# heathsc/bs_call

Measured on AMD Instinct MI355X. Metric: genome positions called/sec, higher is better.
Workload: dtype f64

## Files before the change

### bs_call_amd/csrc/prepdev.hip

```cpp
#include <hip/hip_runtime.h>
#include <stdint.h>

#include "../../include/bscall_amd.h"

#define FLT_QUAL 63u

struct bsc_prep_plan {
  uint64_t src;
  uint64_t ms;
  uint32_t rl0;
  uint32_t w0, wl;
  uint32_t nm;
  uint32_t mark_l, mark_r;
  uint32_t out_len;
  uint32_t present;
  uint32_t trim_l, trim_r;
};

struct bsc_prep_desc {
  uint64_t srcw;
  uint32_t pk;
  int32_t pc;
};
#define PD_PRESENT 1u
// ... 45 lines not shown
  {                                                                                                                                    \
    const uint32_t q = ((w_) >> 2) & 0x3f3f3f3fu;                                                                                      \
    const uint32_t nz = ((q ^ 0x3f3f3f3fu) + 0x7f7f7f7fu) & 0x80808080u;  \
    n += (uint32_t)__popc(nz);                                                                                                         \
    tot = __builtin_amdgcn_sad_u8(q & ((nz >> 7) * 0xffu), 0u, tot);                                       \
  }
  for (; i + 16u <= hi; i += 16u) {
    uint4 v;
    __builtin_memcpy(&v, sp + i, 16);
    MQ_DWORD(v.x) MQ_DWORD(v.y) MQ_DWORD(v.z) MQ_DWORD(v.w)
  }
  for (; i + 4u <= hi; i += 4u) MQ_DWORD(d_ld32(sp + i))
#undef MQ_DWORD
  for (; i < hi; i++) {
    const uint32_t q = (uint32_t)sp[i] >> 2;
    if (q != FLT_QUAL) {
      tot += q;
      n++;
    }
  }
  return n > 0 ? tot / n : 0;
}

__global__ __launch_bounds__(256) void bsc_prep_plan_kernel(const bsc_raw_template *__restrict__ raw, uint32_t nr, const uint8_t *__restrict__ seq,
                                                            uint64_t seq_bytes, const bsc_misms *__restrict__ misms_in, uint64_t n_misms_in,
                                                            bsc_prep_params par, bsc_misms *__restrict__ ms_work,
                                                            bsc_prep_plan *__restrict__ plan, bsc_prep_desc *__restrict__ desc,
                                                            unsigned long long *__restrict__ out_len,
                                                            bsc_template *__restrict__ tpl_out, unsigned long long *__restrict__ cnt,
                                                            uint32_t *__restrict__ max_pos1) {
  const uint32_t ti = blockIdx.x * 256u + threadIdx.x;
  unsigned long long n_clip = 0, n_overlap = 0;
  uint32_t err = 0;
  if (ti < nr) {
    const bsc_raw_template t = raw[ti];
    bsc_prep_plan P[2];
    prep_rd rd[2];
    uint32_t nm[2];
    bsc_misms *ms[2];
    bool edited[2] = {false, false};
    uint32_t pos[2] = {t.pos[0], t.pos[1]};
    if (t.orientation > 1) err = PE_ORI;
#pragma unroll
    for (int k = 0; k < 2 && !err; k++) {
      if (t.len[k] && (t.off[k] > seq_bytes || t.len[k] > seq_bytes - t.off[k])) err = PE_READ + (uint32_t)k;
      else if (t.n_misms[k] && (t.misms_off[k] > n_misms_in || t.n_misms[k] > n_misms_in - t.misms_off[k])) err = PE_LIST + (uint32_t)k;
    }
    if (!err) {
      const int msk = t.orientation == 0 ? 0 : 1;
#pragma unroll
      for (int k = 0; k < 2; k++) {
        const int side = k ^ msk;
        const uint32_t rl = t.len[k];
        const int32_t lt = side ? par.left_trim[1] : par.left_trim[0], rt = side ? par.right_trim[1] : par.right_trim[0];
        P[k].src = t.off[k];
        P[k].ms = t.misms_off[k];
        P[k].rl0 = rl;
        P[k].mark_l = lt > 0 ? ((uint32_t)lt < rl ? (uint32_t)lt : rl) : 0u;
        P[k].mark_r = rt > 0 ? ((uint32_t)rt < rl ? (uint32_t)rt : rl) : 0u;
        P[k].present = rl != 0;
        P[k].trim_l = P[k].trim_r = 0;
        rd[k].w0 = 0;
        rd[k].wl = rl;
        nm[k] = t.n_misms[k];
        ms[k] = ms_work + t.misms_off[k];
        for (uint32_t z = 0; z < nm[k]; z++) ms[k][z] = misms_in[t.misms_off[k] + z];
// ... 174 lines not shown
          }
          m->position = ix1;
        }
        P[k].w0 = rd[k].w0;
        P[k].wl = rl;
        P[k].nm = nm[k];
        P[k].out_len = rl + adj;
      }
    }
    if (err) {
#pragma unroll
      for (int k = 0; k < 2; k++) {
        P[k].src = P[k].ms = 0;
        P[k].rl0 = P[k].w0 = P[k].wl = P[k].nm = P[k].mark_l = P[k].mark_r = P[k].out_len = P[k].present = P[k].trim_l = P[k].trim_r = 0;
      }
      atomicMin(&cnt[0], ((unsigned long long)ti << 8) | err);
      n_clip = n_overlap = 0;
    }
#pragma unroll
    for (int k = 0; k < 2; k++) {
      bsc_prep_desc d;
      const uint32_t ol = P[k].out_len;
      d.srcw = P[k].src + P[k].w0;
      const uint32_t ml = P[k].mark_l > P[k].w0 ? (P[k].mark_l - P[k].w0 < ol ? P[k].mark_l - P[k].w0 : ol) : 0u;
      const uint32_t keep = P[k].rl0 - P[k].mark_r;
      const uint32_t hr = keep > P[k].w0 ? (keep - P[k].w0 < ol ? keep - P[k].w0 : ol) : 0u;
      const bool ed = edited[k] && !err;
      const bool slow = ol != 0 && (ed || hr < ol || ol < 4u || ol >= 0xfffffu || ml >= 256u);
      d.pk = (ol < 0xfffffu ? ol : 0xfffffu) | ((ml & 0xffu) << 20) |
             (((P[k].present ? PD_PRESENT : 0u) | (ed ? PD_EDITED : 0u) | (slow ? PD_SLOW : 0u)) << 28);
      d.pc = k ? (int32_t)(P[k].wl + P[k].trim_r) - 1 : (int32_t)P[k].trim_l;
      desc[2u * ti + (uint32_t)k] = d;
      if (slow) plan[2u * ti + (uint32_t)k] = P[k];
    }
    if (max_pos1) {
      int32_t max_pos = 0;
#pragma unroll
      for (int k = 0; k < 2; k++)
        if (P[k].present) {
          const int32_t mpos = k ? (int32_t)(P[k].wl + P[k].trim_r) - 1 : (int32_t)(P[k].trim_l + P[k].wl);
          if (mpos > max_pos) max_pos = mpos;
        }
      max_pos1[ti] = err ? 0u : (uint32_t)max_pos + 1u;
    }
    out_len[2u * ti] = P[0].out_len;
    out_len[2u * ti + 1u] = P[1].out_len;
    bsc_template o;
    o.pos[0] = pos[0];
    o.pos[1] = pos[1];
    o.len[0] = P[0].out_len;
    o.len[1] = P[1].out_len;
    o.off[0] = o.off[1] = 0;
    o.mapq[0] = t.mapq[0];
    o.mapq[1] = t.mapq[1];
    o.orientation = t.orientation;
    o.bs_strand = t.bs_strand;
    o.flags = 0;
    tpl_out[ti] = o;
  }
  for (int o = 32; o > 0; o >>= 1) {
    n_clip += __shfl_xor(n_clip, o);
    n_overlap += __shfl_xor(n_overlap, o);
  }
  if ((threadIdx.x & 63u) == 0) {
    unsigned long long *slot = cnt + PREP_CNT_WORDS + (blockIdx.x & (PREP_CNT_SLOTS - 1u)) * 8u;
    if (n_clip) atomicAdd(&slot[0], n_clip);
    if (n_overlap) atomicAdd(&slot[1], n_overlap);
  }
}

__device__ static __forceinline__ uint32_t d_marked(const uint8_t *sp, uint32_t i, uint32_t rl0, uint32_t mark_l, uint32_t mark_r) {
  const bool in_r = i >= rl0 - mark_r;
  const uint32_t b = sp[(in_r && 2u * i > rl0 - 1u) ? rl0 - 1u - i : i];
  return (i < mark_l || in_r) ? (b & 3u) | (FLT_QUAL << 2) : (uint32_t)sp[i];
}

struct bsc_prep_prof {
  const uint8_t *ref;
  uint32_t x, n_ref, cap, used0;
  const uint32_t *used_scan;
  unsigned long long *table;
};
__device__ static const uint8_t PROF_REF[64] = {
    0, 0, 0, 0, 0, 0, 0, 0, 0, 0, 0, 8, 0, 0, 0, 0, 0, 4, 4, 0, 4, 0, 0, 0, 0, 0, 0, 8, 0, 0, 0, 0,
    0, 0, 0, 8, 0, 0, 0, 0, 0, 0, 0, 0, 0, 0, 0, 0, 0, 0, 0, 0, 0, 0, 0, 0, 0, 0, 0, 0, 0, 0, 0, 0};
__device__ static __forceinline__ uint32_t d_profile_base(uint32_t bs_strand, uint32_t c) {
  const uint32_t q = c >> 2;
  if (q < 20u  || q >= FLT_QUAL || bs_strand > 2u) return 0u;
  return ((bs_strand == 0 ? 0x7A6Bu : (bs_strand == 1 ? 0x5A4Bu : 0x7869u)) >> (4u * (c & 3u))) & 15u;
}

#define PREP_WAVES 4
#define PREP_BATCH 4u
#define PROF_LDS 512u

__device__ static __forceinline__ void d_prof_base(const bsc_prep_prof &F, uint32_t *s_prof, uint32_t strand, uint32_t used_t, int64_t v,
                                                   int32_t orig, uint32_t byte) {
  const uint32_t xx = d_profile_base(strand, byte);
  if (xx && v + 1 < (int64_t)F.n_ref) {
    const uint32_t ra = v >= 1 ? F.ref[v - 1] : 0u, rb = v >= 0 ? F.ref[v] : 0u, rc = F.ref[v + 1];
    const uint32_t m_before = PROF_REF[((ra << 3) | rb) & 63u], m_after = PROF_REF[((rb << 3) | rc) & 63u];
    if ((((xx & m_after) | ((xx & m_before) >> 1)) >> 2) & 1u) {
      const uint32_t ix = (uint32_t)(orig + 1);
      if (ix < used_t && ix < F.cap) {
        if (ix < PROF_LDS) atomicAdd(&s_prof[(xx & 3u) * PROF_LDS + ix], 1u);
        else atomicAdd(&F.table[(uint64_t)ix * 4u + (xx & 3u)], 1ull);
      }
    }
  }
}

__device__ static __forceinline__ uint32_t d_bcast(uint32_t v, uint32_t l) { return (uint32_t)__builtin_amdgcn_readlane((int)v, (int)l); }
__device__ static __forceinline__ unsigned long long d_bcast64(unsigned long long v, uint32_t l) {
  return (unsigned long long)d_bcast((uint32_t)v, l) | ((unsigned long long)d_bcast((uint32_t)(v >> 32), l) << 32);
}
__device__ static __forceinline__ uint32_t d_ld32(const uint8_t *p) {
  uint32_t v;
  __builtin_memcpy(&v, p, 4);
  return v;
}
__device__ static __forceinline__ void d_st32(uint8_t *p, uint32_t v) { __builtin_memcpy(p, &v, 4); }

struct prep_slow_ret {
  uint32_t c63, cge;
  uint32_t walked;
};

__device__ static __forceinline__ uint32_t prep_slow_src(const bsc_prep_plan &P, const bsc_misms *__restrict__ ms, bool edited, uint32_t j, bool &pad) {
  uint32_t s = j;
  pad = false;
  if (edited) {
    for (uint32_t z = P.nm; z-- > 0;) {
      const bsc_misms m = ms[z];
      if (m.type == BSC_MISMS_INS) {
        if (s >= m.position) {
          if (s - m.position < m.size) {
            pad = true;
            break;
          }
          s -= m.size;
        }
      } else if (m.type == BSC_MISMS_DEL) {
        if (s >= m.position) s += m.size;
      }
    }
  }
  return s;
}

__device__ __noinline__ static prep_slow_ret prep_slow_read(const bsc_prep_plan *__restrict__ plan_r, uint32_t flags, uint8_t *__restrict__ dp,
                                                            const uint8_t *__restrict__ seq, const bsc_misms *__restrict__ ms_work, uint32_t mq) {
  const unsigned lane = threadIdx.x & 63u;
  prep_slow_ret r = {0u, 0u, 0u};
  const bsc_prep_plan P = *plan_r;
  const uint8_t *const sp = seq + P.src;
  const bool edited = (flags & PD_EDITED) != 0;
  if (edited) {
    for (uint32_t s0 = 0; s0 < P.wl; s0 += 64u) {
      const uint32_t s = s0 + lane;
      if (s < P.wl) {
        const uint32_t q = d_marked(sp, P.w0 + s, P.rl0, P.mark_l, P.mark_r) >> 2;
        r.c63 += q == FLT_QUAL;
        r.cge += q >= mq;
      }
    }
  }
  const bsc_misms *const ms = ms_work + P.ms;
  bool walked = false;
  for (uint32_t j0 = 0; j0 < P.out_len; j0 += 64u) {
    const uint32_t j = j0 + lane;
    if (j < P.out_len) {
      bool pad;
      const uint32_t s = prep_slow_src(P, ms, edited, j, pad);
      const uint32_t byte = pad ? 0u : d_marked(sp, P.w0 + s, P.rl0, P.mark_l, P.mark_r);
      const uint32_t q = byte >> 2;
      if (!edited) {
        r.c63 += q == FLT_QUAL;
        r.cge += q >= mq;
      }
      walked |= q != 0 && q != FLT_QUAL;
      dp[j] = (uint8_t)byte;
    }
  }
  r.walked = __any(walked) ? 1u : 0u;
  return r;
}

__global__ __launch_bounds__(64 * PREP_WAVES) void bsc_prep_copy_kernel(const bsc_prep_plan *__restrict__ plan,
                                                                        const bsc_prep_desc *__restrict__ desc, uint32_t nr,
                                                                        const uint8_t *__restrict__ seq, const bsc_misms *__restrict__ ms_work,
                                                                        const unsigned long long *__restrict__ out_off, int32_t min_qual,
                                                                        bsc_template *__restrict__ tpl_out, uint8_t *__restrict__ seq_out,
                                                                        uint64_t seq_out_cap, unsigned long long *__restrict__ cnt) {
  const unsigned lane = threadIdx.x & 63u, lane4 = lane * 4u;
  const uint32_t wave = (uint32_t)__builtin_amdgcn_readfirstlane((int)(blockIdx.x * PREP_WAVES + (threadIdx.x >> 6)));
  const uint32_t n_waves = gridDim.x * PREP_WAVES;
  const uint32_t mq = min_qual < 0 ? 0u : (min_qual > 64 ? 64u : (uint32_t)min_qual), mq4 = mq * 0x01010101u;
  unsigned long long l_total = 0, l_bases = 0;
  uint32_t c63 = 0, cge = 0, l_reads = 0;
  const uint32_t n_reads2 = 2u * nr, n_groups = (n_reads2 + 63u) / 64u;
  for (uint32_t g = wave; g < n_groups; g += n_waves) {
    const uint32_t g0 = g * 64u, n = n_reads2 - g0 < 64u ? n_reads2 - g0 : 64u;
    const uint32_t ri = g0 + (lane < n ? lane : 0u), my_ti = ri >> 1, my_k = ri & 1u;
    bsc_prep_desc L = desc[ri];
    const unsigned long long l_off = out_off[ri];
    if (lane >= n) L.pk = 0;
    if (lane < n) {
      const uint32_t fl = L.pk >> 28;
      uint32_t ol = L.pk & 0xfffffu, wl = ol;
      if (fl & PD_SLOW) {
        ol = plan[ri].out_len;
        wl = plan[ri].wl;
      }
      tpl_out[my_ti].off[my_k] = l_off;
      if (l_off > seq_out_cap || seq_out_cap - l_off < ol) {
        atomicMin(&cnt[0], ((unsigned long long)my_ti << 8) | PE_CAP);
        L.pk &= 0xf0000000u;
      }
      l_total += (fl & PD_EDITED) ? wl : ol;
      if (fl & PD_PRESENT) {
        l_reads++;
        l_bases += wl;
      }
    }
    enum : uint32_t { KIND_LEAN = 1u, KIND_FAST = 2u, KIND_SLOW = 3u };
    const uint32_t my_len = L.pk & 0xfffffu, my_ml = (L.pk >> 20) & 0xffu;
    const uint32_t my_kind = my_len == 0 ? 0u : ((L.pk >> 28) & PD_SLOW ? KIND_SLOW : ((my_len <= 256u && my_ml == 0) ? KIND_LEAN : KIND_FAST));
    const uint32_t l_ctl = (L.pk & 0x0fffffffu) | (my_kind << 28) | (((L.pk >> 28) & PD_EDITED) ? 1u << 30 : 0u);
    const bool my_fetch = my_kind == KIND_LEAN || my_kind == KIND_FAST;
    const unsigned long long l_src = my_fetch ? (unsigned long long)(seq + L.srcw) - (unsigned long long)desc : 0ull;
    unsigned long long walked_mask = 0;
    const unsigned long long obase = d_bcast64(l_off, 0);
    const unsigned long long m_w0 = __ballot(my_kind == KIND_LEAN && my_len >= 16u && my_len <= 128u);
    const unsigned long long sbase = m_w0 ? d_bcast64(L.srcw, (uint32_t)__builtin_ctzll(m_w0)) : 0ull;
// ... 59 lines not shown
        if (ml + 3u > base) {
          const uint32_t nmk = act && ml > o ? (ml - o < 4u ? ml - o : 4u) : 0u;
          const uint32_t mm = nmk >= 4u ? 0xffffffffu : (1u << (8u * nmk)) - 1u;
          w = (w & ~mm) | (((w & 0x03030303u) | 0xfcfcfcfcu) & mm);
        }
        const uint32_t wc = act ? w >> (8u * (nominal - o)) : 0u;
        const uint32_t qh = ((wc >> 2) & 0x3f3f3f3fu) | 0x80808080u;
        const uint32_t q1 = qh + 0x01010101u;
        c63 += (uint32_t)__popc(q1 & 0x40404040u);
        cge += (uint32_t)__popc((qh - mq4) & 0x80808080u);
        if (k == 0) walked |= __any((q1 & 0x3e3e3e3eu) != 0u) != 0;
        if (act) d_st32(dp + o, w);
      }
      if (k == 0 && walked) walked_mask |= 1ull << l;
    };
    if (__ballot(my_wide)) {
      uint4 va[RW], vb[RW];
      fetch8(0, va);
#pragma unroll
      for (uint32_t i0 = 0; i0 < 8u; i0 += 2u * RW) {
        fetch8(i0 + RW, vb);
        process8(i0, va);
        fetch8(i0 + 2u * RW, va);
        process8(i0 + RW, vb);
      }
      walk_bits |= (uint32_t)__shfl_xor((int)walk_bits, 1);
      walk_bits |= (uint32_t)__shfl_xor((int)walk_bits, 2);
      walk_bits |= (uint32_t)__shfl_xor((int)walk_bits, 4);
      walked_mask |= __ballot((walk_bits >> (lane & 7u)) & 1u);
    }
    for (unsigned long long rest = __ballot(my_kind != 0u && !my_wide); rest; rest &= rest - 1ull) one((uint32_t)__builtin_ctzll(rest));
    if (lane < n && my_k == 0) tpl_out[my_ti].flags = BSC_TPL_WALK_KNOWN | (((walked_mask >> lane) & 1ull) ? BSC_TPL_WALKED0 : 0u);
  }
  unsigned long long w[5] = {l_total, c63, cge, l_reads, l_bases};
  for (int i = 0; i < 5; i++)
    for (int o = 32; o > 0; o >>= 1) w[i] += __shfl_xor(w[i], o);
  if (mq == 0) w[2] = w[0];
  if (lane == 0) {
    const unsigned long long low = w[0] - w[2] - (mq > FLT_QUAL ? w[1] : 0ull), none = w[0] - w[1] - low;
    if (none) atomicAdd(&cnt[3], none);
    if (w[1]) atomicAdd(&cnt[4], w[1]);
    if (low) atomicAdd(&cnt[5], low);
    if (w[3]) atomicAdd(&cnt[6], w[3]);
    if (w[4]) atomicAdd(&cnt[7], w[4]);
  }
}

__global__ __launch_bounds__(256) void bsc_prep_refmask_kernel(const uint8_t *__restrict__ ref, uint32_t n_ref, uint8_t *__restrict__ mask) {
  const uint64_t i = ((uint64_t)blockIdx.x * 256u + threadIdx.x) * 4u;
  if (i >= (uint64_t)n_ref + 24u) return;
  uint32_t m = 0;
  if (i >= 12u && i - 8u + 7u <= n_ref) {
    const uint64_t v = i - 8u;
    const uint32_t lo = d_ld32(ref + v - 1u) & 0x07070707u, hi = d_ld32(ref + v + 3u) & 0x07070707u;
    const uint32_t r_at = __builtin_amdgcn_alignbyte(hi, lo, 1u), r_next = __builtin_amdgcn_alignbyte(hi, lo, 2u);
#define PROF_NE(x, c) ((((x) ^ ((c) * 0x01010101u)) + 0x7f7f7f7fu) & 0x80808080u)
    const uint32_t over_c = ~PROF_NE(r_at, 2u) & PROF_NE(r_next, 0u) & PROF_NE(r_next, 3u) & 0x80808080u;
    const uint32_t over_g = ~PROF_NE(r_at, 3u) & PROF_NE(lo, 0u) & PROF_NE(lo, 2u) & 0x80808080u;
#undef PROF_NE
    m = (over_c >> 5) | (over_g >> 4);
  } else {
    for (uint32_t t = 0; t < 4u; t++) {
      const uint64_t it = i + t;
      if (it >= 8u && it - 8u + 1u < n_ref) {
        const uint64_t v = it - 8u;
        const uint32_t ra = v >= 1 ? ref[v - 1] : 0u, rb = ref[v], rc = ref[v + 1];
        m |= ((PROF_REF[((rb << 3) | rc) & 63u] & 4u) | (PROF_REF[((ra << 3) | rb) & 63u] & 8u)) << (8u * t);
      }
    }
  }
  __builtin_memcpy(mask + i, &m, 4);
}

__global__ __launch_bounds__(64 * PREP_WAVES) void bsc_prep_profile_kernel(const bsc_prep_plan *__restrict__ plan, const bsc_prep_desc *__restrict__ desc,
                                                                           uint32_t nr, const bsc_misms *__restrict__ ms_work,
                                                                           const unsigned long long *__restrict__ out_off,
                                                                           const bsc_template *__restrict__ tpl_out, const uint8_t *__restrict__ seq_out,
                                                                           uint64_t seq_out_cap, unsigned long long *__restrict__ cnt,
                                                                           const uint8_t *__restrict__ mask, const bsc_prep_prof F) {
  __shared__ uint32_t s_prof[PROF_LDS * 4u];
  for (unsigned i = threadIdx.x; i < PROF_LDS * 4u; i += 64 * PREP_WAVES) s_prof[i] = 0;
  __syncthreads();
  const unsigned lane = threadIdx.x & 63u;
  const uint32_t wave = (uint32_t)__builtin_amdgcn_readfirstlane((int)(blockIdx.x * PREP_WAVES + (threadIdx.x >> 6)));
  const uint32_t n_waves = gridDim.x * PREP_WAVES;
  const uint32_t n_reads2 = 2u * nr, n_groups = (n_reads2 + 63u) / 64u;
  uint32_t acc[4][2] = {{0u, 0u}, {0u, 0u}, {0u, 0u}, {0u, 0u}};
  uint32_t acc_n = 0;
  bool acc_quarter = true;
  auto flush = [&]() {
    const uint32_t p0 = 8u * (acc_quarter ? (lane & 15u) : (lane & 31u));
#pragma unroll
    for (uint32_t b = 0; b < 4u; b++) {
      const uint32_t col = (0x63u >> (2u * b)) & 3u;
#pragma unroll
      for (uint32_t t = 0; t < 8u; t++) {
        const uint32_t c = (acc[b][t >> 2] >> (8u * (t & 3u))) & 0xffu;
        if (c) atomicAdd(&s_prof[col * PROF_LDS + p0 + t + 1u], c);
      }
      acc[b][0] = acc[b][1] = 0u;
    }
    acc_n = 0;
  };
  for (uint32_t g = wave; g < n_groups; g += n_waves) {
    const uint32_t g0 = g * 64u, n = n_reads2 - g0 < 64u ? n_reads2 - g0 : 64u;
    const uint32_t ri = g0 + (lane < n ? lane : 0u), my_ti = ri >> 1, my_k = ri & 1u;
    const bsc_prep_desc L = desc[ri];
    const unsigned long long l_off = out_off[ri];
    const uint32_t us_prev = my_ti ? F.used_scan[my_ti - 1u] : 0u, us_mine = F.used_scan[my_ti];
    const uint32_t t_strand = tpl_out[my_ti].bs_strand, t_pos = tpl_out[my_ti].pos[my_k];
    uint32_t c1 = 0, kind = 0, l_used = 0, l_strand = 0, l_ol = 0, top = 0;
    if (lane < n) {
      const uint32_t fl = L.pk >> 28;
      uint32_t ol = L.pk & 0xfffffu;
      if (fl & PD_SLOW) ol = plan[ri].out_len;
      const bool fits = !(l_off > seq_out_cap || seq_out_cap - l_off < ol);
      if ((fl & PD_PRESENT) && ol != 0 && fits) {
        const uint32_t before = my_ti ? (us_prev > F.used0 ? us_prev : F.used0) : F.used0;
        l_used = us_mine > before ? us_mine : before;
        if (l_used > before && (unsigned long long)l_used + 1ull > F.cap) atomicMin(&cnt[0], ((unsigned long long)my_ti << 8) | PE_PROF_CAP);
        l_strand = t_strand;
        const uint32_t pos = t_pos;
        l_ol = ol;
        const bool in_ref = pos >= F.x && (uint64_t)pos - F.x + ol + 1u <= F.n_ref;
        if (!in_ref) atomicMin(&cnt[0], ((unsigned long long)my_ti << 8) | PE_PROF_RANGE);
        if (in_ref && l_strand <= 2u) {
          const uint32_t lim = l_used < F.cap ? l_used : F.cap;
          const int32_t pc = L.pc;
          top = my_k ? (uint32_t)(pc < 0 ? 0 : pc) : (uint32_t)pc + ol - 1u;
          const bool regs = !(fl & PD_SLOW) && l_strand != 0u && ol <= 256u && pc >= 0 && pc < 512 && top < 256u && top + 1u < lim && l_off >= 8u &&
                            seq_out_cap - l_off - ol >= 8u;
          kind = regs ? 1u : 2u;
          c1 = pos > F.x ? pos - F.x + 1u : 0u;
        }
      }
    }
    unsigned long long m_regs = __ballot(kind == 1u);
    if (m_regs) {
      const uint32_t first = (uint32_t)__builtin_ctzll(m_regs);
      const unsigned long long obase = d_bcast64(l_off, first);
      const unsigned long long orel = l_off - obase;
      if (kind == 1u && orel >= (1ull << 15)) kind = 2u;
      const uint32_t A1 = kind == 1u ? (c1 + 7u) | (l_strand == 2u ? 1u << 29 : 0u) | (1u << 31) : 0u;
      const uint32_t A2 = kind == 1u ? (l_ol - 1u) | ((uint32_t)L.pc << 8) | ((uint32_t)orel << 17) : 0u;
      const bool quarter = __ballot(kind == 1u && top >= 128u) == 0ull;
      if (quarter != acc_quarter) {
        flush();
        acc_quarter = quarter;
      }
      const uint8_t *const sb = seq_out + obase - 8u;
      const uint32_t h = quarter ? (lane & 15u) : (lane & 31u);
      const int32_t p0 = (int32_t)(8u * h);
      const uint32_t hsel = quarter ? (lane & 48u) : (lane & 32u), rounds = quarter ? 16u : 32u;
      constexpr uint32_t B = 2u;
      struct rnd {
        uint32_t a1;
        unsigned long long w, mw;
        int32_t jc, len8;
      };
      auto ask = [&](uint32_t i, rnd &r) {
        const int src = (int)(hsel | (i & (rounds - 1u)));
        r.a1 = (uint32_t)__shfl((int)A1, src);
        const uint32_t a2 = (uint32_t)__shfl((int)A2, src);
        const int32_t len = (int32_t)(a2 & 0xffu) + 1;
        r.len8 = 8 - len;
        const int32_t pc = (int32_t)((a2 >> 8) & 0x1ffu);
        const int32_t j0 = (i & 1u) ? pc - p0 - 7 : p0 - pc;
        const bool some = (int32_t)r.a1 < 0 && (uint32_t)(j0 + 7) < (uint32_t)(len + 7);
        r.jc = some ? j0 : 0;
        __builtin_memcpy(&r.w, sb + ((a2 >> 17) + (uint32_t)(r.jc + 8)), 8);
        __builtin_memcpy(&r.mw, mask + (some ? (r.a1 & 0x1fffffffu) + (uint32_t)j0 : 0u), 8);
      };
      auto count = [&](uint32_t i, const rnd &r) {
        const int32_t lo = r.jc < 0 ? -r.jc : 0, hi = r.jc + r.len8 > 0 ? r.jc + r.len8 : 0;
        unsigned long long w8 = r.w & (~0ull << (8 * lo)) & (~0ull >> (8 * hi));
        unsigned long long m8 = r.mw;
        if (i & 1u) {
          w8 = __builtin_bswap64(w8);
          m8 = __builtin_bswap64(m8);
        }
        const uint32_t sx = (r.a1 >> 29) & 1u ? 0xffffffffu : 0u;
#pragma unroll
        for (int d = 0; d < 2; d++) {
          const uint32_t w = (uint32_t)(w8 >> (32 * d)), mw = (uint32_t)(m8 >> (32 * d));
          const uint32_t odd = w << 7;
          const uint32_t qf = ((w >> 2) & 0x3f3f3f3fu) | 0x80808080u;
          const uint32_t q_ok = (qf - 20u * 0x01010101u) & ~((qf + 0x01010101u) << 1) & 0x80808080u;
          const uint32_t hb = (((odd & (mw << 5)) | (~odd & (mw << 4))) & q_ok) >> 7;
          const uint32_t wb = w ^ sx;
          const uint32_t t1 = hb & (wb >> 1), t0 = hb ^ t1, t3 = t1 & wb, t2 = t0 & wb;
          acc[3][d] += t3;
          acc[2][d] += t1 ^ t3;
          acc[1][d] += t2;
          acc[0][d] += t0 ^ t2;
        }
      };
      rnd ra[B], rb[B];
#pragma unroll
      for (uint32_t u = 0; u < B; u++) ask(u, ra[u]);
      for (uint32_t i0 = 0; i0 < rounds; i0 += 2u * B) {
        if (acc_n + 2u * B > 255u) flush();
#pragma unroll
        for (uint32_t u = 0; u < B; u++) ask(i0 + B + u, rb[u]);
#pragma unroll
        for (uint32_t u = 0; u < B; u++) count(u, ra[u]);
#pragma unroll
        for (uint32_t u = 0; u < B; u++) ask(i0 + 2u * B + u, ra[u]);
#pragma unroll
        for (uint32_t u = 0; u < B; u++) count(B + u, rb[u]);
        acc_n += 2u * B;
      }
    }
    unsigned long long m_long = __ballot(kind == 2u);
    while (m_long) {
      const uint32_t l = (uint32_t)__builtin_ctzll(m_long);
      m_long &= m_long - 1ull;
      const uint32_t ol = d_bcast(l_ol, l), k = l & 1u, strand = d_bcast(l_strand, l), used_t = d_bcast(l_used, l);
      const int32_t pc = (int32_t)d_bcast((uint32_t)L.pc, l);
      const int64_t v0 = (int64_t)d_bcast(c1, l) - 1;
      const uint8_t *const dp = seq_out + d_bcast64(l_off, l);
      const bool slow = (d_bcast(L.pk, l) >> 28) & PD_SLOW;
      bsc_prep_plan P;
      bool edited = false;
      if (slow) {
        P = plan[g0 + l];
        edited = (d_bcast(L.pk, l) >> 28) & PD_EDITED;
      }
      for (uint32_t jb = 0; jb < ol; jb += 64u) {
        const uint32_t j = jb + lane;
        if (j < ol) {
          bool pad = false;
          const uint32_t s = slow ? prep_slow_src(P, ms_work + P.ms, edited, j, pad) : j;
          if (!pad) d_prof_base(F, s_prof, strand, used_t, v0 + j, k ? pc - (int32_t)s : pc + (int32_t)s, dp[j]);
        }
      }
    }
  }
  flush();
  __syncthreads();
  for (unsigned i = threadIdx.x; i < PROF_LDS * 4u; i += 64 * PREP_WAVES)
    if (s_prof[i] && i % PROF_LDS < F.cap) atomicAdd(&F.table[(uint64_t)(i % PROF_LDS) * 4u + i / PROF_LDS], (unsigned long long)s_prof[i]);
}

extern "C" int bsc_dev_scan_u64(const void *in, void *out, uint32_t n, void *tmp, size_t tmp_bytes, void *stream);

extern "C" size_t bsc_dev_prep_plan_bytes(void) { return sizeof(bsc_prep_plan) + sizeof(bsc_prep_desc); }

extern "C" int bsc_dev_scan_max_u32(const void *in, void *out, uint32_t n, void *tmp, size_t tmp_bytes, void *stream);

extern "C" int bsc_dev_launch_prep(const void *raw, uint32_t nr, const void *seq, uint64_t seq_bytes, const void *misms, uint64_t n_misms,
                                   const bsc_prep_params *par, void *ms_work, void *plan, void *out_len, void *out_off, void *scan_tmp,
                                   size_t scan_tmp_bytes, void *tpl_out, void *seq_out, uint64_t seq_out_cap, void *cnt, int num_cus,
                                   void *stream, const void *prof_ref, uint32_t prof_x, uint32_t prof_n_ref, uint32_t prof_cap,
                                   uint32_t prof_used0, void *prof_table, void *max_pos1, void *used_scan, void *prof_mask) {
  hipStream_t s = (hipStream_t)stream;
  bsc_prep_desc *const desc = (bsc_prep_desc *)((bsc_prep_plan *)plan + 2ull * nr);
  if (!nr) return (int)hipMemsetAsync(out_off, 0, sizeof(unsigned long long), s);
  hipError_t e = hipMemsetAsync((unsigned long long *)out_len + 2ull * nr, 0, sizeof(unsigned long long), s);
  if (e != hipSuccess) return (int)e;
  hipLaunchKernelGGL(bsc_prep_plan_kernel, dim3((nr + 255u) / 256u), dim3(256), 0, s, (const bsc_raw_template *)raw, nr, (const uint8_t *)seq,
                     seq_bytes, (const bsc_misms *)misms, n_misms, *par, (bsc_misms *)ms_work, (bsc_prep_plan *)plan, desc,
                     (unsigned long long *)out_len, (bsc_template *)tpl_out, (unsigned long long *)cnt, prof_ref ? (uint32_t *)max_pos1 : nullptr);
  if ((e = hipGetLastError()) != hipSuccess) return (int)e;
  int rc = bsc_dev_scan_u64(out_len, out_off, 2u * nr + 1u, scan_tmp, scan_tmp_bytes, stream);
  if (rc) return rc;
  bsc_prep_prof F = {nullptr, 0u, 0u, 0u, 0u, nullptr, nullptr};
  if (prof_ref) {
    if ((rc = bsc_dev_scan_max_u32(max_pos1, used_scan, nr, scan_tmp, scan_tmp_bytes, stream))) return rc;
    F.ref = (const uint8_t *)prof_ref;
    F.x = prof_x;
    F.n_ref = prof_n_ref;
    F.cap = prof_cap;
    F.used0 = prof_used0;
    F.used_scan = (const uint32_t *)used_scan;
    F.table = (unsigned long long *)prof_table;
  }
  unsigned g = ((nr + 31u) / 32u + PREP_WAVES - 1u) / PREP_WAVES;
  static int per_cu[2] = {0, 0};
  for (int pv = 0; pv < (prof_ref ? 2 : 1); pv++)
    if (!per_cu[pv]) {
      int nb = 0;
      const hipError_t eo = pv ? hipOccupancyMaxActiveBlocksPerMultiprocessor(&nb, bsc_prep_profile_kernel, 64 * PREP_WAVES, 0)
                               : hipOccupancyMaxActiveBlocksPerMultiprocessor(&nb, bsc_prep_copy_kernel, 64 * PREP_WAVES, 0);
      per_cu[pv] = (eo == hipSuccess && nb > 0) ? nb : 4;
      (void)hipGetLastError();
    }
  unsigned gc = g, gp = g;
  if (gc > (unsigned)num_cus * (unsigned)per_cu[0]) gc = (unsigned)num_cus * (unsigned)per_cu[0];
  hipLaunchKernelGGL(bsc_prep_copy_kernel, dim3(gc), dim3(64 * PREP_WAVES), 0, s, (const bsc_prep_plan *)plan, (const bsc_prep_desc *)desc, nr,
                     (const uint8_t *)seq, (const bsc_misms *)ms_work, (const unsigned long long *)out_off, par->min_qual, (bsc_template *)tpl_out,
                     (uint8_t *)seq_out, seq_out_cap, (unsigned long long *)cnt);
  if ((e = hipGetLastError()) != hipSuccess) return (int)e;
  if (prof_ref) {
    hipLaunchKernelGGL(bsc_prep_refmask_kernel, dim3((unsigned)(((uint64_t)prof_n_ref + 24u + 1023u) / 1024u)), dim3(256), 0, s, (const uint8_t *)prof_ref,
                       prof_n_ref, (uint8_t *)prof_mask);
    if ((e = hipGetLastError()) != hipSuccess) return (int)e;
    if (gp > (unsigned)num_cus * (unsigned)per_cu[1]) gp = (unsigned)num_cus * (unsigned)per_cu[1];
    hipLaunchKernelGGL(bsc_prep_profile_kernel, dim3(gp), dim3(64 * PREP_WAVES), 0, s, (const bsc_prep_plan *)plan, (const bsc_prep_desc *)desc, nr,
                       (const bsc_misms *)ms_work, (const unsigned long long *)out_off, (const bsc_template *)tpl_out, (const uint8_t *)seq_out,
                       seq_out_cap, (unsigned long long *)cnt, (const uint8_t *)prof_mask, F);
  }
  return (int)hipGetLastError();
}
```

Baseline: 17.90 billion.

## Fuse read copy with fast-path profiling and split slow reads into separate kernel

After: 17.90 billion (median of 4 runs). About the same (+0.0%).

```diff
diff --git a/bs_call_amd/csrc/prepdev.hip b/bs_call_amd/csrc/prepdev.hip
--- a/bs_call_amd/csrc/prepdev.hip
+++ b/bs_call_amd/csrc/prepdev.hip
@@ -101,6 +101,7 @@
   const uint32_t ti = blockIdx.x * 256u + threadIdx.x;
   unsigned long long n_clip = 0, n_overlap = 0;
   uint32_t err = 0;
+  bool slow_k[2] = {false, false};
   if (ti < nr) {
     const bsc_raw_template t = raw[ti];
     bsc_prep_plan P[2];
@@ -341,6 +342,7 @@
       d.pc = k ? (int32_t)(P[k].wl + P[k].trim_r) - 1 : (int32_t)P[k].trim_l;
       desc[2u * ti + (uint32_t)k] = d;
       if (slow) plan[2u * ti + (uint32_t)k] = P[k];
+      slow_k[k] = slow;
     }
     if (max_pos1) {
       int32_t max_pos = 0;
@@ -371,10 +373,12 @@
     n_clip += __shfl_xor(n_clip, o);
     n_overlap += __shfl_xor(n_overlap, o);
   }
+  const uint32_t n_slow = (uint32_t)__popcll(__ballot(slow_k[0])) + (uint32_t)__popcll(__ballot(slow_k[1]));
   if ((threadIdx.x & 63u) == 0) {
     unsigned long long *slot = cnt + PREP_CNT_WORDS + (blockIdx.x & (PREP_CNT_SLOTS - 1u)) * 8u;
     if (n_clip) atomicAdd(&slot[0], n_clip);
     if (n_overlap) atomicAdd(&slot[1], n_overlap);
+    if (n_slow) atomicAdd(&slot[2], (unsigned long long)n_slow);
   }
 }
 
@@ -400,21 +404,19 @@
 }
 
 #define PREP_WAVES 4
+#define PREP_PROF_WAVES 4
+#define PREP_SLOW_WAVES 16
 #define PREP_BATCH 4u
 #define PROF_LDS 512u
 
-__device__ static __forceinline__ void d_prof_base(const bsc_prep_prof &F, uint32_t *s_prof, uint32_t strand, uint32_t used_t, int64_t v,
-                                                   int32_t orig, uint32_t byte) {
+__device__ static __forceinline__ void d_prof_count(const bsc_prep_prof &F, uint32_t *s_prof, uint32_t strand, uint32_t used_t, uint32_t m, int32_t orig,
+                                                    uint32_t byte) {
   const uint32_t xx = d_profile_base(strand, byte);
-  if (xx && v + 1 < (int64_t)F.n_ref) {
-    const uint32_t ra = v >= 1 ? F.ref[v - 1] : 0u, rb = v >= 0 ? F.ref[v] : 0u, rc = F.ref[v + 1];
-    const uint32_t m_before = PROF_REF[((ra << 3) | rb) & 63u], m_after = PROF_REF[((rb << 3) | rc) & 63u];
-    if ((((xx & m_after) | ((xx & m_before) >> 1)) >> 2) & 1u) {
-      const uint32_t ix = (uint32_t)(orig + 1);
-      if (ix < used_t && ix < F.cap) {
-        if (ix < PROF_LDS) atomicAdd(&s_prof[(xx & 3u) * PROF_LDS + ix], 1u);
-        else atomicAdd(&F.table[(uint64_t)ix * 4u + (xx & 3u)], 1ull);
-      }
+  if (xx & m & 12u) {
+    const uint32_t ix = (uint32_t)(orig + 1);
+    if (ix < used_t && ix < F.cap) {
+      if (ix < PROF_LDS) atomicAdd(&s_prof[(xx & 3u) * PROF_LDS + ix], 1u);
+      else atomicAdd(&F.table[(uint64_t)ix * 4u + (xx & 3u)], 1ull);
     }
   }
 }
@@ -448,6 +450,32 @@
             break;
           }
           s -= m.size;
+        }
+      } else if (m.type == BSC_MISMS_DEL) {
+        if (s >= m.position) s += m.size;
+      }
+    }
+  }
+  return s;
+}
+
+__device__ static __forceinline__ uint32_t prep_slow_src_regs(const bsc_misms *__restrict__ ms, const uint32_t nm, const bsc_misms &mine, bool edited,
+                                                              uint32_t j, bool &pad) {
+  uint32_t s = j;
+  pad = false;
+  if (edited) {
+    for (uint32_t z = nm; z-- > 0;) {
+      bsc_misms m;
+      if (z < 64u) {
+        m.type = d_bcast(mine.type, z);
+        m.position = d_bcast(mine.position, z);
+        m.size = d_bcast(mine.size, z);
+      } else m = ms[z];
+      if (pad) continue;
+      if (m.type == BSC_MISMS_INS) {
+        if (s >= m.position) {
+          if (s - m.position < m.size) pad = true;
+          else s -= m.size;
         }
       } else if (m.type == BSC_MISMS_DEL) {
         if (s >= m.position) s += m.size;
@@ -495,20 +523,21 @@
   return r;
 }
 
-__global__ __launch_bounds__(64 * PREP_WAVES) void bsc_prep_copy_kernel(const bsc_prep_plan *__restrict__ plan,
-                                                                        const bsc_prep_desc *__restrict__ desc, uint32_t nr,
-                                                                        const uint8_t *__restrict__ seq, const bsc_misms *__restrict__ ms_work,
-                                                                        const unsigned long long *__restrict__ out_off, int32_t min_qual,
-                                                                        bsc_template *__restrict__ tpl_out, uint8_t *__restrict__ seq_out,
-                                                                        uint64_t seq_out_cap, unsigned long long *__restrict__ cnt) {
+struct prep_copy_sums {
+  unsigned long long l_total, l_bases;
+  uint32_t c63, cge, l_reads;
+};
+
+__device__ static __forceinline__ void prep_copy_group(const uint32_t g, const uint32_t n_reads2, const bsc_prep_plan *__restrict__ plan,
+                                                       const bsc_prep_desc *__restrict__ desc, const uint8_t *__restrict__ seq,
+                                                       const bsc_misms *__restrict__ ms_work, const unsigned long long *__restrict__ out_off,
+                                                       const uint32_t mq, bsc_template *__restrict__ tpl_out, uint8_t *__restrict__ seq_out,
+                                                       const uint64_t seq_out_cap, unsigned long long *__restrict__ cnt, prep_copy_sums &S) {
   const unsigned lane = threadIdx.x & 63u, lane4 = lane * 4u;
-  const uint32_t wave = (uint32_t)__builtin_amdgcn_readfirstlane((int)(blockIdx.x * PREP_WAVES + (threadIdx.x >> 6)));
-  const uint32_t n_waves = gridDim.x * PREP_WAVES;
-  const uint32_t mq = min_qual < 0 ? 0u : (min_qual > 64 ? 64u : (uint32_t)min_qual), mq4 = mq * 0x01010101u;
-  unsigned long long l_total = 0, l_bases = 0;
-  uint32_t c63 = 0, cge = 0, l_reads = 0;
-  const uint32_t n_reads2 = 2u * nr, n_groups = (n_reads2 + 63u) / 64u;
-  for (uint32_t g = wave; g < n_groups; g += n_waves) {
+  const uint32_t mq4 = mq * 0x01010101u;
+  unsigned long long &l_total = S.l_total, &l_bases = S.l_bases;
+  uint32_t &c63 = S.c63, &cge = S.cge, &l_reads = S.l_reads;
+  {
     const uint32_t g0 = g * 64u, n = n_reads2 - g0 < 64u ? n_reads2 - g0 : 64u;
     const uint32_t ri = g0 + (lane < n ? lane : 0u), my_ti = ri >> 1, my_k = ri & 1u;
     bsc_prep_desc L = desc[ri];
@@ -634,7 +663,11 @@
     for (unsigned long long rest = __ballot(my_kind != 0u && !my_wide); rest; rest &= rest - 1ull) one((uint32_t)__builtin_ctzll(rest));
     if (lane < n && my_k == 0) tpl_out[my_ti].flags = BSC_TPL_WALK_KNOWN | (((walked_mask >> lane) & 1ull) ? BSC_TPL_WALKED0 : 0u);
   }
-  unsigned long long w[5] = {l_total, c63, cge, l_reads, l_bases};
+}
+
+__device__ static __forceinline__ void prep_copy_finish(const prep_copy_sums &S, const uint32_t mq, unsigned long long *__restrict__ cnt) {
+  const unsigned lane = threadIdx.x & 63u;
+  unsigned long long w[5] = {S.l_total, S.c63, S.cge, S.l_reads, S.l_bases};
   for (int i = 0; i < 5; i++)
     for (int o = 32; o > 0; o >>= 1) w[i] += __shfl_xor(w[i], o);
   if (mq == 0) w[2] = w[0];
@@ -674,48 +707,62 @@
   __builtin_memcpy(mask + i, &m, 4);
 }
 
-__global__ __launch_bounds__(64 * PREP_WAVES) void bsc_prep_profile_kernel(const bsc_prep_plan *__restrict__ plan, const bsc_prep_desc *__restrict__ desc,
-                                                                           uint32_t nr, const bsc_misms *__restrict__ ms_work,
-                                                                           const unsigned long long *__restrict__ out_off,
-                                                                           const bsc_template *__restrict__ tpl_out, const uint8_t *__restrict__ seq_out,
-                                                                           uint64_t seq_out_cap, unsigned long long *__restrict__ cnt,
-                                                                           const uint8_t *__restrict__ mask, const bsc_prep_prof F) {
-  __shared__ uint32_t s_prof[PROF_LDS * 4u];
-  for (unsigned i = threadIdx.x; i < PROF_LDS * 4u; i += 64 * PREP_WAVES) s_prof[i] = 0;
-  __syncthreads();
+struct prep_prof_regs {
+  uint32_t acc[4][2];
+  uint32_t acc_n;
+  bool acc_quarter;
+};
+__device__ static __forceinline__ void prep_prof_flush(prep_prof_regs &R, uint32_t *s_prof) {
   const unsigned lane = threadIdx.x & 63u;
-  const uint32_t wave = (uint32_t)__builtin_amdgcn_readfirstlane((int)(blockIdx.x * PREP_WAVES + (threadIdx.x >> 6)));
-  const uint32_t n_waves = gridDim.x * PREP_WAVES;
-  const uint32_t n_reads2 = 2u * nr, n_groups = (n_reads2 + 63u) / 64u;
-  uint32_t acc[4][2] = {{0u, 0u}, {0u, 0u}, {0u, 0u}, {0u, 0u}};
-  uint32_t acc_n = 0;
-  bool acc_quarter = true;
-  auto flush = [&]() {
-    const uint32_t p0 = 8u * (acc_quarter ? (lane & 15u) : (lane & 31u));
-#pragma unroll
-    for (uint32_t b = 0; b < 4u; b++) {
-      const uint32_t col = (0x63u >> (2u * b)) & 3u;
-#pragma unroll
-      for (uint32_t t = 0; t < 8u; t++) {
-        const uint32_t c = (acc[b][t >> 2] >> (8u * (t & 3u))) & 0xffu;
-        if (c) atomicAdd(&s_prof[col * PROF_LDS + p0 + t + 1u], c);
-      }
-      acc[b][0] = acc[b][1] = 0u;
-    }
-    acc_n = 0;
-  };
-  for (uint32_t g = wave; g < n_groups; g += n_waves) {
+  const uint32_t p0 = 8u * (R.acc_quarter ? (lane & 15u) : (lane & 31u));
+#pragma unroll
+  for (uint32_t b = 0; b < 4u; b++) {
+    const uint32_t col = (0x63u >> (2u * b)) & 3u;
+#pragma unroll
+    for (uint32_t t = 0; t < 8u; t++) {
+      const uint32_t c = (R.acc[b][t >> 2] >> (8u * (t & 3u))) & 0xffu;
+      if (c) atomicAdd(&s_prof[col * PROF_LDS + p0 + t + 1u], c);
+    }
+    R.acc[b][0] = R.acc[b][1] = 0u;
+  }
+  R.acc_n = 0;
+}
+__device__ static __forceinline__ void prep_prof_table_out(const uint32_t *s_prof, const bsc_prep_prof &F) {
+  for (unsigned i = threadIdx.x; i < PROF_LDS * 4u; i += blockDim.x)
+    if (s_prof[i] && i % PROF_LDS < F.cap) atomicAdd(&F.table[(uint64_t)(i % PROF_LDS) * 4u + i / PROF_LDS], (unsigned long long)s_prof[i]);
+}
+
+template <bool RAW>
+__device__ static __forceinline__ void prep_profile_group(const uint32_t g, const uint32_t n_reads2, const bsc_prep_plan *__restrict__ plan,
+                                                          const bsc_prep_desc *__restrict__ desc, const bsc_misms *__restrict__ ms_work,
+                                                          const unsigned long long *__restrict__ out_off, const bsc_template *tpl_out,
+                                                          const uint8_t *bytes, const uint64_t bytes_n, const uint64_t seq_out_cap,
+                                                          unsigned long long *__restrict__ cnt, const uint8_t *__restrict__ mask, const bsc_prep_prof &F,
+                                                          uint32_t *s_prof, prep_prof_regs &R) {
+  const unsigned lane = threadIdx.x & 63u;
+  uint32_t(&acc)[4][2] = R.acc;
+  uint32_t &acc_n = R.acc_n;
+  bool &acc_quarter = R.acc_quarter;
+  auto flush = [&]() { prep_prof_flush(R, s_prof); };
+  {
     const uint32_t g0 = g * 64u, n = n_reads2 - g0 < 64u ? n_reads2 - g0 : 64u;
     const uint32_t ri = g0 + (lane < n ? lane : 0u), my_ti = ri >> 1, my_k = ri & 1u;
     const bsc_prep_desc L = desc[ri];
+    if (!RAW && !__ballot(lane < n && ((L.pk >> 28) & PD_SLOW))) return;
     const unsigned long long l_off = out_off[ri];
     const uint32_t us_prev = my_ti ? F.used_scan[my_ti - 1u] : 0u, us_mine = F.used_scan[my_ti];
     const uint32_t t_strand = tpl_out[my_ti].bs_strand, t_pos = tpl_out[my_ti].pos[my_k];
     uint32_t c1 = 0, kind = 0, l_used = 0, l_strand = 0, l_ol = 0, top = 0;
-    if (lane < n) {
+    uint32_t l_nm = 0;
+    unsigned long long l_ms = 0;
+    if (lane < n && (((L.pk >> 28) & PD_SLOW) != 0u) == !RAW) {
       const uint32_t fl = L.pk >> 28;
       uint32_t ol = L.pk & 0xfffffu;
-      if (fl & PD_SLOW) ol = plan[ri].out_len;
+      if (!RAW) {
+        ol = plan[ri].out_len;
+        l_nm = plan[ri].nm;
+        l_ms = plan[ri].ms;
+      }
       const bool fits = !(l_off > seq_out_cap || seq_out_cap - l_off < ol);
       if ((fl & PD_PRESENT) && ol != 0 && fits) {
         const uint32_t before = my_ti ? (us_prev > F.used0 ? us_prev : F.used0) : F.used0;
@@ -730,27 +777,28 @@
           const uint32_t lim = l_used < F.cap ? l_used : F.cap;
           const int32_t pc = L.pc;
           top = my_k ? (uint32_t)(pc < 0 ? 0 : pc) : (uint32_t)pc + ol - 1u;
-          const bool regs = !(fl & PD_SLOW) && l_strand != 0u && ol <= 256u && pc >= 0 && pc < 512 && top < 256u && top + 1u < lim && l_off >= 8u &&
-                            seq_out_cap - l_off - ol >= 8u;
+          const bool regs = RAW && l_strand != 0u && ol <= 256u && pc >= 0 && pc < 512 && top < 256u && top + 1u < lim && L.srcw >= 8u &&
+                            bytes_n - L.srcw - ol >= 8u;
           kind = regs ? 1u : 2u;
           c1 = pos > F.x ? pos - F.x + 1u : 0u;
         }
       }
     }
-    unsigned long long m_regs = __ballot(kind == 1u);
+    unsigned long long m_regs = RAW ? __ballot(kind == 1u) : 0ull;
     if (m_regs) {
       const uint32_t first = (uint32_t)__builtin_ctzll(m_regs);
-      const unsigned long long obase = d_bcast64(l_off, first);
-      const unsigned long long orel = l_off - obase;
-      if (kind == 1u && orel >= (1ull << 15)) kind = 2u;
+      const unsigned long long sbase = d_bcast64(L.srcw, first);
+      const unsigned long long srel = L.srcw - sbase;
+      if (kind == 1u && srel >= (1ull << 31)) kind = 2u;
       const uint32_t A1 = kind == 1u ? (c1 + 7u) | (l_strand == 2u ? 1u << 29 : 0u) | (1u << 31) : 0u;
-      const uint32_t A2 = kind == 1u ? (l_ol - 1u) | ((uint32_t)L.pc << 8) | ((uint32_t)orel << 17) : 0u;
+      const uint32_t A2 = kind == 1u ? (l_ol - 1u) | ((uint32_t)L.pc << 8) | (((L.pk >> 20) & 0xffu) << 17) : 0u;
+      const uint32_t A3 = kind == 1u ? (uint32_t)srel : 0u;
       const bool quarter = __ballot(kind == 1u && top >= 128u) == 0ull;
       if (quarter != acc_quarter) {
         flush();
         acc_quarter = quarter;
       }
-      const uint8_t *const sb = seq_out + obase - 8u;
+      const uint8_t *const sb = bytes + sbase - 8u;
       const uint32_t h = quarter ? (lane & 15u) : (lane & 31u);
       const int32_t p0 = (int32_t)(8u * h);
       const uint32_t hsel = quarter ? (lane & 48u) : (lane & 32u), rounds = quarter ? 16u : 32u;
@@ -758,24 +806,25 @@
       struct rnd {
         uint32_t a1;
         unsigned long long w, mw;
-        int32_t jc, len8;
+        int32_t lo, hi;
       };
       auto ask = [&](uint32_t i, rnd &r) {
         const int src = (int)(hsel | (i & (rounds - 1u)));
         r.a1 = (uint32_t)__shfl((int)A1, src);
         const uint32_t a2 = (uint32_t)__shfl((int)A2, src);
-        const int32_t len = (int32_t)(a2 & 0xffu) + 1;
-        r.len8 = 8 - len;
+        const uint32_t a3 = (uint32_t)__shfl((int)A3, src);
+        const int32_t len = (int32_t)(a2 & 0xffu) + 1, ml = (int32_t)((a2 >> 17) & 0xffu);
         const int32_t pc = (int32_t)((a2 >> 8) & 0x1ffu);
         const int32_t j0 = (i & 1u) ? pc - p0 - 7 : p0 - pc;
         const bool some = (int32_t)r.a1 < 0 && (uint32_t)(j0 + 7) < (uint32_t)(len + 7);
-        r.jc = some ? j0 : 0;
-        __builtin_memcpy(&r.w, sb + ((a2 >> 17) + (uint32_t)(r.jc + 8)), 8);
+        const int32_t jc = some ? j0 : 0, below = ml - jc, behind = jc + 8 - len;
+        r.lo = below < 0 ? 0 : (below > 8 ? 8 : below);
+        r.hi = behind > 0 ? behind : 0;
+        __builtin_memcpy(&r.w, sb + (a3 + (uint32_t)(jc + 8)), 8);
         __builtin_memcpy(&r.mw, mask + (some ? (r.a1 & 0x1fffffffu) + (uint32_t)j0 : 0u), 8);
       };
       auto count = [&](uint32_t i, const rnd &r) {
-        const int32_t lo = r.jc < 0 ? -r.jc : 0, hi = r.jc + r.len8 > 0 ? r.jc + r.len8 : 0;
-        unsigned long long w8 = r.w & (~0ull << (8 * lo)) & (~0ull >> (8 * hi));
+        unsigned long long w8 = r.w & ((~0ull << (4 * r.lo)) << (4 * r.lo)) & (~0ull >> (8 * r.hi));
         unsigned long long m8 = r.mw;
         if (i & 1u) {
           w8 = __builtin_bswap64(w8);
@@ -820,28 +869,91 @@
       const uint32_t ol = d_bcast(l_ol, l), k = l & 1u, strand = d_bcast(l_strand, l), used_t = d_bcast(l_used, l);
       const int32_t pc = (int32_t)d_bcast((uint32_t)L.pc, l);
       const int64_t v0 = (int64_t)d_bcast(c1, l) - 1;
-      const uint8_t *const dp = seq_out + d_bcast64(l_off, l);
-      const bool slow = (d_bcast(L.pk, l) >> 28) & PD_SLOW;
-      bsc_prep_plan P;
-      bool edited = false;
-      if (slow) {
-        P = plan[g0 + l];
-        edited = (d_bcast(L.pk, l) >> 28) & PD_EDITED;
-      }
-      for (uint32_t jb = 0; jb < ol; jb += 64u) {
-        const uint32_t j = jb + lane;
-        if (j < ol) {
+      const uint8_t *const dp = bytes + (RAW ? d_bcast64(L.srcw, l) : d_bcast64(l_off, l));
+      const uint32_t ml = RAW ? (d_bcast(L.pk, l) >> 20) & 0xffu : 0u;
+      const bool edited = !RAW && ((d_bcast(L.pk, l) >> 28) & PD_EDITED);
+      const uint32_t nm = d_bcast(l_nm, l);
+      const bsc_misms *const ms = ms_work + d_bcast64(l_ms, l);
+      bsc_misms mine = {0u, 0u, 0u};
+      if (edited && lane < nm) mine = ms[lane];
+      for (uint32_t jb = 0; jb < ol; jb += 256u) {
+        uint32_t byt[4], mk[4];
+#pragma unroll
+        for (uint32_t u = 0; u < 4u; u++) {
+          const uint32_t j = jb + 64u * u + lane;
+          byt[u] = j < ol ? (uint32_t)dp[j] : 0u;
+          mk[u] = j < ol ? (uint32_t)mask[(uint64_t)(v0 + 8 + (int64_t)j)] : 0u;
+        }
+#pragma unroll
+        for (uint32_t u = 0; u < 4u; u++) {
+          const uint32_t j = jb + 64u * u + lane;
           bool pad = false;
-          const uint32_t s = slow ? prep_slow_src(P, ms_work + P.ms, edited, j, pad) : j;
-          if (!pad) d_prof_base(F, s_prof, strand, used_t, v0 + j, k ? pc - (int32_t)s : pc + (int32_t)s, dp[j]);
-        }
-      }
-    }
-  }
-  flush();
+          const uint32_t s = !RAW ? prep_slow_src_regs(ms, nm, mine, edited, j, pad) : j;
+          const uint32_t byte = RAW && j < ml ? (byt[u] & 3u) | (FLT_QUAL << 2) : byt[u];
+          if (j < ol && !pad) d_prof_count(F, s_prof, strand, used_t, mk[u], k ? pc - (int32_t)s : pc + (int32_t)s, byte);
+        }
+      }
+    }
+  }
+}
+
+__global__ __launch_bounds__(64 * PREP_WAVES) void bsc_prep_copy_kernel(const bsc_prep_plan *__restrict__ plan,
+                                                                        const bsc_prep_desc *__restrict__ desc, uint32_t nr,
+                                                                        const uint8_t *__restrict__ seq, const bsc_misms *__restrict__ ms_work,
+                                                                        const unsigned long long *__restrict__ out_off, int32_t min_qual,
+                                                                        bsc_template *__restrict__ tpl_out, uint8_t *__restrict__ seq_out,
+                                                                        uint64_t seq_out_cap, unsigned long long *__restrict__ cnt) {
+  const uint32_t wave = (uint32_t)__builtin_amdgcn_readfirstlane((int)(blockIdx.x * PREP_WAVES + (threadIdx.x >> 6)));
+  const uint32_t n_waves = gridDim.x * PREP_WAVES;
+  const uint32_t mq = min_qual < 0 ? 0u : (min_qual > 64 ? 64u : (uint32_t)min_qual);
+  const uint32_t n_reads2 = 2u * nr, n_groups = (n_reads2 + 63u) / 64u;
+  prep_copy_sums S = {0ull, 0ull, 0u, 0u, 0u};
+  for (uint32_t g = wave; g < n_groups; g += n_waves) prep_copy_group(g, n_reads2, plan, desc, seq, ms_work, out_off, mq, tpl_out, seq_out, seq_out_cap, cnt, S);
+  prep_copy_finish(S, mq, cnt);
+}
+
+__global__ __launch_bounds__(64 * PREP_PROF_WAVES) __attribute__((amdgpu_waves_per_eu(5))) void bsc_prep_copy_profile_kernel(
+    const bsc_prep_plan *__restrict__ plan, const bsc_prep_desc *__restrict__ desc, uint32_t nr, const uint8_t *__restrict__ seq, uint64_t seq_bytes,
+    const bsc_misms *__restrict__ ms_work, const unsigned long long *__restrict__ out_off, int32_t min_qual, bsc_template *tpl_out,
+    uint8_t *__restrict__ seq_out, uint64_t seq_out_cap, unsigned long long *__restrict__ cnt, const uint8_t *__restrict__ mask, const bsc_prep_prof F) {
+  __shared__ uint32_t s_prof[PROF_LDS * 4u];
+  for (unsigned i = threadIdx.x; i < PROF_LDS * 4u; i += 64 * PREP_PROF_WAVES) s_prof[i] = 0;
   __syncthreads();
-  for (unsigned i = threadIdx.x; i < PROF_LDS * 4u; i += 64 * PREP_WAVES)
-    if (s_prof[i] && i % PROF_LDS < F.cap) atomicAdd(&F.table[(uint64_t)(i % PROF_LDS) * 4u + i / PROF_LDS], (unsigned long long)s_prof[i]);
+  const uint32_t wave = (uint32_t)__builtin_amdgcn_readfirstlane((int)(blockIdx.x * PREP_PROF_WAVES + (threadIdx.x >> 6)));
+  const uint32_t n_waves = gridDim.x * PREP_PROF_WAVES;
+  const uint32_t mq = min_qual < 0 ? 0u : (min_qual > 64 ? 64u : (uint32_t)min_qual);
+  const uint32_t n_reads2 = 2u * nr, n_groups = (n_reads2 + 63u) / 64u;
+  prep_copy_sums S = {0ull, 0ull, 0u, 0u, 0u};
+  prep_prof_regs R = {{{0u, 0u}, {0u, 0u}, {0u, 0u}, {0u, 0u}}, 0u, true};
+  for (uint32_t g = wave; g < n_groups; g += n_waves) {
+    prep_copy_group(g, n_reads2, plan, desc, seq, ms_work, out_off, mq, tpl_out, seq_out, seq_out_cap, cnt, S);
+    prep_profile_group<true>(g, n_reads2, plan, desc, ms_work, out_off, tpl_out, seq, seq_bytes, seq_out_cap, cnt, mask, F, s_prof, R);
+  }
+  prep_prof_flush(R, s_prof);
+  __syncthreads();
+  prep_prof_table_out(s_prof, F);
+  prep_copy_finish(S, mq, cnt);
+}
+
+__global__ __launch_bounds__(64 * PREP_SLOW_WAVES) void bsc_prep_profile_kernel(const bsc_prep_plan *__restrict__ plan, const bsc_prep_desc *__restrict__ desc,
+                                                                           uint32_t nr, const bsc_misms *__restrict__ ms_work,
+                                                                           const unsigned long long *__restrict__ out_off,
+                                                                           const bsc_template *__restrict__ tpl_out, const uint8_t *__restrict__ seq_out,
+                                                                           uint64_t seq_out_cap, unsigned long long *__restrict__ cnt,
+                                                                           const uint8_t *__restrict__ mask, const bsc_prep_prof F) {
+  __shared__ uint32_t s_prof[PROF_LDS * 4u];
+  const unsigned lane = threadIdx.x & 63u;
+  if (!__ballot(cnt[PREP_CNT_WORDS + lane * 8u + 2u] != 0ull)) return;
+  for (unsigned i = threadIdx.x; i < PROF_LDS * 4u; i += 64 * PREP_SLOW_WAVES) s_prof[i] = 0;
+  __syncthreads();
+  const uint32_t wave = (uint32_t)__builtin_amdgcn_readfirstlane((int)(blockIdx.x * PREP_SLOW_WAVES + (threadIdx.x >> 6)));
+  const uint32_t n_waves = gridDim.x * PREP_SLOW_WAVES;
+  const uint32_t n_reads2 = 2u * nr, n_groups = (n_reads2 + 63u) / 64u;
+  prep_prof_regs R = {{{0u, 0u}, {0u, 0u}, {0u, 0u}, {0u, 0u}}, 0u, true};
+  for (uint32_t g = wave; g < n_groups; g += n_waves)
+    prep_profile_group<false>(g, n_reads2, plan, desc, ms_work, out_off, tpl_out, seq_out, seq_out_cap, seq_out_cap, cnt, mask, F, s_prof, R);
+  __syncthreads();
+  prep_prof_table_out(s_prof, F);
 }
 
 extern "C" int bsc_dev_scan_u64(const void *in, void *out, uint32_t n, void *tmp, size_t tmp_bytes, void *stream);
@@ -877,30 +989,37 @@
     F.used_scan = (const uint32_t *)used_scan;
     F.table = (unsigned long long *)prof_table;
   }
-  unsigned g = ((nr + 31u) / 32u + PREP_WAVES - 1u) / PREP_WAVES;
-  static int per_cu[2] = {0, 0};
-  for (int pv = 0; pv < (prof_ref ? 2 : 1); pv++)
+  const unsigned n_groups = (nr + 31u) / 32u;
+  static int per_cu[3] = {0, 0, 0};
+  for (int pv = 0; pv < (prof_ref ? 3 : 1); pv++)
     if (!per_cu[pv]) {
       int nb = 0;
-      const hipError_t eo = pv ? hipOccupancyMaxActiveBlocksPerMultiprocessor(&nb, bsc_prep_profile_kernel, 64 * PREP_WAVES, 0)
-                               : hipOccupancyMaxActiveBlocksPerMultiprocessor(&nb, bsc_prep_copy_kernel, 64 * PREP_WAVES, 0);
-      per_cu[pv] = (eo == hipSuccess && nb > 0) ? nb : 4;
+      const hipError_t eo = pv == 0   ? hipOccupancyMaxActiveBlocksPerMultiprocessor(&nb, bsc_prep_copy_kernel, 64 * PREP_WAVES, 0)
+                            : pv == 1 ? hipOccupancyMaxActiveBlocksPerMultiprocessor(&nb, bsc_prep_copy_profile_kernel, 64 * PREP_PROF_WAVES, 0)
+                                      : hipOccupancyMaxActiveBlocksPerMultiprocessor(&nb, bsc_prep_profile_kernel, 64 * PREP_SLOW_WAVES, 0);
+      per_cu[pv] = (eo == hipSuccess && nb > 0) ? nb : (pv == 0 ? 4 : 1);
       (void)hipGetLastError();
     }
-  unsigned gc = g, gp = g;
-  if (gc > (unsigned)num_cus * (unsigned)per_cu[0]) gc = (unsigned)num_cus * (unsigned)per_cu[0];
-  hipLaunchKernelGGL(bsc_prep_copy_kernel, dim3(gc), dim3(64 * PREP_WAVES), 0, s, (const bsc_prep_plan *)plan, (const bsc_prep_desc *)desc, nr,
-                     (const uint8_t *)seq, (const bsc_misms *)ms_work, (const unsigned long long *)out_off, par->min_qual, (bsc_template *)tpl_out,
-                     (uint8_t *)seq_out, seq_out_cap, (unsigned long long *)cnt);
+  const unsigned wg_waves = prof_ref ? PREP_PROF_WAVES : PREP_WAVES;
+  unsigned gc = (n_groups + wg_waves - 1u) / wg_waves, gp = (n_groups + PREP_SLOW_WAVES - 1u) / PREP_SLOW_WAVES;
+  const unsigned per_copy = (unsigned)per_cu[prof_ref ? 1 : 0];
+  if (gc > (unsigned)num_cus * per_copy) gc = (unsigned)num_cus * per_copy;
+  if (!prof_ref) {
+    hipLaunchKernelGGL(bsc_prep_copy_kernel, dim3(gc), dim3(64 * PREP_WAVES), 0, s, (const bsc_prep_plan *)plan, (const bsc_prep_desc *)desc, nr,
+                       (const uint8_t *)seq, (const bsc_misms *)ms_work, (const unsigned long long *)out_off, par->min_qual,
+                       (bsc_template *)tpl_out, (uint8_t *)seq_out, seq_out_cap, (unsigned long long *)cnt);
+    return (int)hipGetLastError();
+  }
+  hipLaunchKernelGGL(bsc_prep_refmask_kernel, dim3((unsigned)(((uint64_t)prof_n_ref + 24u + 1023u) / 1024u)), dim3(256), 0, s, (const uint8_t *)prof_ref,
+                     prof_n_ref, (uint8_t *)prof_mask);
   if ((e = hipGetLastError()) != hipSuccess) return (int)e;
-  if (prof_ref) {
-    hipLaunchKernelGGL(bsc_prep_refmask_kernel, dim3((unsigned)(((uint64_t)prof_n_ref + 24u + 1023u) / 1024u)), dim3(256), 0, s, (const uint8_t *)prof_ref,
-                       prof_n_ref, (uint8_t *)prof_mask);
-    if ((e = hipGetLastError()) != hipSuccess) return (int)e;
-    if (gp > (unsigned)num_cus * (unsigned)per_cu[1]) gp = (unsigned)num_cus * (unsigned)per_cu[1];
-    hipLaunchKernelGGL(bsc_prep_profile_kernel, dim3(gp), dim3(64 * PREP_WAVES), 0, s, (const bsc_prep_plan *)plan, (const bsc_prep_desc *)desc, nr,
-                       (const bsc_misms *)ms_work, (const unsigned long long *)out_off, (const bsc_template *)tpl_out, (const uint8_t *)seq_out,
-                       seq_out_cap, (unsigned long long *)cnt, (const uint8_t *)prof_mask, F);
-  }
+  hipLaunchKernelGGL(bsc_prep_copy_profile_kernel, dim3(gc), dim3(64 * PREP_PROF_WAVES), 0, s, (const bsc_prep_plan *)plan, (const bsc_prep_desc *)desc, nr,
+                     (const uint8_t *)seq, seq_bytes, (const bsc_misms *)ms_work, (const unsigned long long *)out_off, par->min_qual,
+                     (bsc_template *)tpl_out, (uint8_t *)seq_out, seq_out_cap, (unsigned long long *)cnt, (const uint8_t *)prof_mask, F);
+  if ((e = hipGetLastError()) != hipSuccess) return (int)e;
+  if (gp > (unsigned)num_cus * (unsigned)per_cu[2]) gp = (unsigned)num_cus * (unsigned)per_cu[2];
+  hipLaunchKernelGGL(bsc_prep_profile_kernel, dim3(gp), dim3(64 * PREP_SLOW_WAVES), 0, s, (const bsc_prep_plan *)plan, (const bsc_prep_desc *)desc, nr,
+                     (const bsc_misms *)ms_work, (const unsigned long long *)out_off, (const bsc_template *)tpl_out, (const uint8_t *)seq_out,
+                     seq_out_cap, (unsigned long long *)cnt, (const uint8_t *)prof_mask, F);
   return (int)hipGetLastError();
 }
```
